# jjalcaraz-upct/network-slicing

Hardware: AMD Instinct MI355X
Metric: env-steps/sec (batched RanSlice.step, scenario_0) (higher is better)
Workload: dtype f64

## Files before the change

network-slicing_amd/csrc/rs_api.hip:

```cpp

#include <hip/hip_runtime.h>

#include <cmath>
#include <cstdio>
#include <cstdlib>
#include <cstring>
#include <string>
#include <vector>

#include "rs_host.h"

#ifdef RS_DEV
static inline const char* dev_env(const char* name) { return getenv(name); }
#else
static inline const char* dev_env(const char*) { return nullptr; }
#endif

#include "rs_embb.hip"
#include "rs_mmtc.hip"
#include "rs_order.hip"
#include "rs_mux.hip"

using namespace rs;

// ... 285 lines not shown
    for (int k = 0; k < 4; ++k) atomicAdd(&acc[k], loc[k]);
    __syncthreads();
    if (threadIdx.x < 4) atomicAdd((unsigned long long*)&out[threadIdx.x], acc[threadIdx.x]);
}

}


static void mcs_factors(double* A, double* B) {
    double Delta = 0.1;
    double a = 1.0 / Delta;
    double s01 = rs_sigmoid(0.1, 0.0, 1.0), s09 = rs_sigmoid(0.9, 0.0, 1.0);
    a = a * (rs_log(1.0 / s01 - 1.0) - rs_log(1.0 / s09 - 1.0));
    *A = a;
    *B = -rs_log(1.0 / s09 - 1.0);
}

static void mcs_lookup(const rs_config* c, double A, double B, int e_snr, int* mcs_out, int* rate_out) {
    double rx_prob = 1.0 - 0.1;
    int mcs;
    for (mcs = 0; mcs < c->n_mcs; ++mcs) {
        double x = A * ((double)e_snr - c->mcs_snr[mcs]) - B;
        if (rs_sigmoid(x, 0.0, 1.0) < rx_prob) {
            *mcs_out = mcs - 1 > 0 ? mcs - 1 : 0;
            *rate_out = (int)((double)c->sym_per_prb * (c->mcs_rate[mcs] * (double)c->mcs_order[mcs]));
            return;
        }
    }
    mcs = c->n_mcs - 1;
    *mcs_out = mcs;
    *rate_out = (int)((double)c->sym_per_prb * (c->mcs_rate[mcs] * (double)c->mcs_order[mcs]));
}

static void rx_fast_setup(RsDev& d, double* band0) {
    const double A = d.mcsA;
    double kmax = 0.0, kmin = 1e300;
    bool ok = std::isfinite(A) && A > 0.0 && std::isfinite(d.mcsB);
    for (int m = 0; m < 3; ++m) {
        const double k = d.mi_k[m];
        ok = ok && std::isfinite(k) && k > 0.0 && std::isfinite(d.mi_x0[m]);
        kmax = k > kmax ? k : kmax;
        kmin = k < kmin ? k : kmin;
        d.rx_c1[m] = (float)(-k * RS_INV_LN2);
    }
    ok = ok && A / kmax >= 1.0 && A / kmin <= 1.0e4;
    d.rx_invA = ok ? (float)(1.0 / A) : 0.0f;
    d.rx_B = (float)d.mcsB;
    d.rx_band = 0.0;
    *band0 = ok ? 6.0e-6 + 6.0e-6 * (kmax / A) : 0.0;
    d.rx_band1 = ok ? 4.0e-5 / A + 1.0e-6 : 0.0;
    if (dev_env("RANSLICE_RX_EXACT")) *band0 = 0.0;
    if (const char* e = dev_env("RANSLICE_RX_BAND_SCALE")) {
        const double f = atof(e);
        if (f >= 1.0) d.rx_band1 *= f;
    }
}

extern "C" int rs_create(const rs_config* cfg, int device, rs_handle** out) {
    if (!cfg || !out) return RS_EINVAL;
    *out = nullptr;
    rs_handle* h = new rs_handle();
    *out = h;
    h->cfg = *cfg;
    h->device = device;
    if (cfg->n_envs <= 0 || cfg->n_prbs <= 0 || cfg->n_prbs > RS_MAX_PRBS || cfg->n_embb < 0 || cfg->n_mmtc < 0 ||
        cfg->n_embb + cfg->n_mmtc <= 0 || cfg->slots_per_step <= 0 || cfg->slots_per_step > 63 || cfg->n_mcs <= 0 || cfg->n_mcs > 32 ||
// ... 280 lines not shown
        vbytes += h->valid_host[f].size();
        bool any_valid = false;
        for (uint8_t v : h->valid_host[f]) {
            if (!v) d.has_nan = 1;
            any_valid = any_valid || v;
        }
        if (!any_valid) {
            h->err = "rs_load_fading: a trace has no NaN-free column";
            return RS_EINVAL;
        }
    }
    if (elems + (size_t)RS_MAX_PRBS >= (size_t)1 << 31) {
        h->err = "rs_load_fading: tables exceed 2^31 samples";
        return RS_EINVAL;
    }
    if (h->fad) (void)hipFree(h->fad);
    if (h->fad_valid) (void)hipFree(h->fad_valid);
    if (h->fad32) (void)hipFree(h->fad32);
    if (h->fps) (void)hipFree(h->fps);
    h->fad32 = nullptr;
    h->fps = nullptr;
    HIPCHK(h, hipMalloc((void**)&h->fad, sizeof(double) * (elems + 16)));
    HIPCHK(h, hipMalloc((void**)&h->fad_valid, vbytes + 16));
    if (const char* v = dev_env("RANSLICE_GUARD"))
        if (v[0] == '2') fprintf(stderr, "RANSLICE_GUARD: fading table at %p, %zu bytes\n", (void*)h->fad, sizeof(double) * (elems + 16));
    for (int f = 0; f < RS_N_TRACES; ++f) {
        HIPCHK(h, hipMemcpyAsync(h->fad + d.fad_off[f], h->fad_host[f].data(), sizeof(double) * h->fad_host[f].size(),
                                 hipMemcpyHostToDevice, h->stream));
        HIPCHK(h, hipMemcpyAsync(h->fad_valid + d.valid_off[f], h->valid_host[f].data(), h->valid_host[f].size(),
                                 hipMemcpyHostToDevice, h->stream));
    }
    {
        const int P = d.P;
        std::vector<float> t32(elems + 64, 0.0f);
        std::vector<double> ps((elems / (size_t)P) * (size_t)(P + 1) + 16, 0.0);
        double smax = 0.0;
        bool finite = true;
        for (int f = 0; f < RS_N_TRACES; ++f) {
            const std::vector<double>& tab = h->fad_host[f];
            const size_t cols = tab.size() / (size_t)P, c0 = (size_t)d.fad_off[f] / (size_t)P;
            d.col_off[f] = (int32_t)c0;
            for (size_t t = 0; t < cols; ++t) {
                long double acc = 0.0L;
                double* row = &ps[(c0 + t) * (size_t)(P + 1)];
                row[0] = 0.0;
                const bool ok = h->valid_host[f][t] != 0;
                for (int p = 0; p < P; ++p) {
                    const double v = tab[t * (size_t)P + p];
                    t32[(size_t)d.fad_off[f] + t * (size_t)P + p] = (float)v;
                    acc += (long double)v;
                    row[p + 1] = (double)acc;
                    if (ok) {
                        finite = finite && std::isfinite(v);
                        smax = std::fabs(v) > smax ? std::fabs(v) : smax;
                    }
                }
            }
        }
        const bool small = finite && smax <= 1.0e3;
        const bool ps_fits = ps.size() + (size_t)RS_MAX_PRBS < ((size_t)1 << 31);
        d.est_band = (small && ps_fits && !dev_env("RANSLICE_EST_EXACT")) ? 1.0e-9 : 0.0;
        double kmax = 0.0;
        for (int m = 0; m < 3; ++m) kmax = d.mi_k[m] > kmax ? d.mi_k[m] : kmax;
        d.rx_band = (small && h->rx_band0 > 0.0) ? h->rx_band0 + 0.5 * kmax * 5.97e-8 * smax : 0.0;
        if (const char* e = dev_env("RANSLICE_RX_BAND_SCALE")) {
            const double fsc = atof(e);
            if (fsc >= 1.0) d.rx_band *= fsc;
        }
        if (const char* e = dev_env("RANSLICE_EST_BAND")) {
            const double b = atof(e);
            if (d.est_band > 0.0 && b > 0.0 && b < 0.5) d.est_band = b;
        }
        HIPCHK(h, hipMalloc((void**)&h->fad32, sizeof(float) * t32.size()));
        HIPCHK(h, hipMalloc((void**)&h->fps, sizeof(double) * ps.size()));
        HIPCHK(h, hipMemcpy(h->fad32, t32.data(), sizeof(float) * t32.size(), hipMemcpyHostToDevice));
        HIPCHK(h, hipMemcpy(h->fps, ps.data(), sizeof(double) * ps.size(), hipMemcpyHostToDevice));
    }
    HIPCHK(h, hipMemcpyAsync(h->ddev, &d, sizeof d, hipMemcpyHostToDevice, h->stream));
    HIPCHK(h, hipStreamSynchronize(h->stream));
    h->fad_hash = fading_hash(h);
    for (int f = 0; f < RS_N_TRACES; ++f) {
        std::vector<double>().swap(h->fad_host[f]);
        std::vector<uint8_t>().swap(h->valid_host[f]);
    }
    return RS_OK;
}

extern "C" int rs_load_fading(rs_handle* h, int trace_id, const double* data, int rows, int cols) {
    if (!h) return RS_EINVAL;
    if (trace_id < 0 || trace_id >= RS_N_TRACES || !data || rows <= 0 || cols <= 0 || h->cfg.n_prbs > 2 * rows) {
        h->err = "rs_load_fading: bad arguments";
        return RS_EINVAL;
    }
    HIPCHK(h, hipSetDevice(h->device));
    drop_graph(h);
    if (h->tables_borrowed) {
        h->err = "rs_load_fading: a lookahead branch handle shares its tables";
        return RS_ESTATE;
    }
    if (h->la) {
        HIPCHK(h, hipStreamSynchronize(h->stream));
        rs_destroy(h->la);
        h->la = nullptr;
    }
    h->fad_hash = 0;
    const int P = h->cfg.n_prbs > rows ? h->cfg.n_prbs : rows;
    if (h->hdev.P != 0 && h->hdev.P != P) {
        h->err = "rs_load_fading: all traces must have the same number of rows";
// ... 610 lines not shown
```

network-slicing_amd/csrc/rs_device.h:

```cpp
#pragma once
#include <stdint.h>

#define RS_GROUP 32
#define RS_BURSTS 16
#define RS_BURST_MAX_LEN 16000
#define RS_LUT_MAX 64
#define RS_NEVER 0x7fffffff
#define RS_MAX_PRBS 256

#define rs_burst_code(end_abs) (0x8000u | ((unsigned)(end_abs) & 0x7fffu))
#define rs_burst_rel(code, now) ((int)(((((unsigned)(code)) - (unsigned)(now)) & 0x7fffu) ^ 0x4000u) - 0x4000)

struct RsDev {
    int32_t n_envs, n_prbs, n_embb, n_mmtc, n_slices, slots, n_vars;
    int32_t n_act;
    int32_t mux;
    int32_t P;
    int32_t T[3];
    int32_t has_nan;
    int64_t fad_off[3];
    int64_t valid_off[3];
    double slot_length;
    double cbr_bits;
    double cbr_ia_scale, cbr_hold_scale;
    double vbr_ia_scale, vbr_hold_scale;
    double vbr_p_size, vbr_b_size, vbr_inter;
    double sla[6], norm[10];
    double prop_A, prop_B;
    double mcsA, mcsB;
    double pf_a, pf_b;
    double slot_rc;
    int32_t pf_div_fast;
    int32_t gran;
    int32_t lut_lo, lut_n;
    int32_t lut_mcs[RS_LUT_MAX], lut_rate[RS_LUT_MAX];
    double mcs_ref[32];
    int32_t mcs_mod[32];
    double mi_x0[3], mi_k[3];
    double rx_band;
    double est_band;
    int32_t col_off[3];
    int32_t pad_rx;
    double rx_band1;
    float rx_c1[3];
    float rx_invA, rx_B;
    double penalty;
    int32_t mtc_n_dev, mtc_cap, mtc_n_rep, mtc_n_period;
    int32_t mtc_rep_set[8], mtc_period_set[8];
    double sla_mtc_delay, norm_mmtc[3];
};

struct RsState {
    int32_t* t_n_ue;
    int32_t* t_cbr_at;
    int32_t* t_vbr_at;
    uint32_t* t_ctr;
    uint32_t* t_serial;
    int32_t* t_cost;
    double* u_queue;
    double* u_th;
    double* u_nominal;
    int32_t* u_hold_at;
    int32_t* u_e_snr;
    int32_t* u_findex;
    int32_t* u_bits;
    int32_t* u_prbs;
    int32_t* u_vbr_at;
    uint32_t* u_ctr;
    uint32_t* u_serial;
    int32_t* u_flags;
    uint16_t* u_burst;
    uint64_t* seeds;
    int32_t* err;
};
```

network-slicing_amd/csrc/rs_embb.hip:

```cpp

#pragma once
#include <hip/hip_runtime.h>
#include <stdint.h>

#include "rs_device.h"

#if defined(__HIP_DEVICE_COMPILE__)
__device__ double rs_exp_ool(double x);
__device__ double rs_log_ool(double x);
#define RS_EXP_CALL rs_exp_ool
#define RS_LOG_CALL rs_log_ool
#endif
#include "../../include/rs_philox.h"
#include "../../include/ranslice.h"

typedef double rs_d2 __attribute__((ext_vector_type(2)));
#if defined(__HIP_DEVICE_COMPILE__)
__device__ __noinline__ double rs_exp_ool(double x) { return rs_exp(x); }
__device__ __noinline__ double rs_log_ool(double x) { return rs_log(x); }
__device__ __forceinline__ double rs_exp_sel(double x, double core) {
    double v = x < -745.2 ? 0.0 : core;
    v = x > 709.782712893384 ? rs_inf() : v;
    return x != x ? x : v;
}
// ... 73 lines not shown
#define SEC_FLUSH(buf)                                                                                  \
    if ((threadIdx.x & 63u) == 0u) {                                                                    \
        unsigned long long tot_ = 0;                                                                    \
        for (int i_ = 0; i_ < 13; ++i_) tot_ += sec_acc[i_];                                            \
        for (int i_ = 0; i_ < 16; ++i_)                                                                 \
            if (i_ != 14) atomicAdd((unsigned long long*)&(buf)[i_], sec_acc[i_]);                      \
         \
        if (tot_ > atomicMax((unsigned long long*)&(buf)[14], tot_))                                    \
            for (int i_ = 0; i_ < 16; ++i_) (buf)[16 + 4 * (size_t)n_tasks + i_] = sec_acc[i_];        \
    }                                                                                                   \
    if ((threadIdx.x & 63u) != 0u && sec_acc[13]) atomicAdd((unsigned long long*)&(buf)[13], sec_acc[13]); \
    if (gl == 0 && valid) {  \
        unsigned long long tot_ = 0;                                                                    \
        for (int i_ = 0; i_ < 13; ++i_) tot_ += sec_acc[i_];                                            \
        (buf)[16 + task * 4 + 0] = tot_;                                                                \
         \
        (buf)[16 + task * 4 + 1] = (unsigned long long)S.t_n_ue[task] |                                 \
                                   ((unsigned long long)__builtin_amdgcn_s_getreg(63508) << 32);        \
        (buf)[16 + task * 4 + 2] = (unsigned long long)A.actions[rep * n_slices + sl] |                 \
                                   ((unsigned long long)__builtin_amdgcn_s_getreg(63492) << 32);        \
        (buf)[16 + task * 4 + 3] = (unsigned long long)(stat >> 18) | ((sec_t0 - tot_) << 24);  \
    }
#else
#define SEC_DECL
#define SEC_MARK(i)
#define SEC_FLUSH(buf)
#endif

__device__ __forceinline__ int bperm(int v, int src_lane) {
    return __builtin_amdgcn_ds_bpermute(src_lane << 2, v);
}
__device__ __forceinline__ unsigned bperm(unsigned v, int src_lane) {
    return (unsigned)__builtin_amdgcn_ds_bpermute(src_lane << 2, (int)v);
}
__device__ __forceinline__ double bperm(double v, int src_lane) {
    uint64_t u = rs_d2u(v);
    int lo = __builtin_amdgcn_ds_bpermute(src_lane << 2, (int)(uint32_t)u);
    int hi = __builtin_amdgcn_ds_bpermute(src_lane << 2, (int)(uint32_t)(u >> 32));
    return rs_u2d(((uint64_t)(uint32_t)hi << 32) | (uint32_t)lo);
}

__device__ __forceinline__ bool wave_any(bool c) { return __builtin_amdgcn_ballot_w64(c) != 0ull; }

#define DPP_XOR1 0xB1
#define DPP_XOR2 0x4E
#define DPP_HMIRROR 0x141
#define DPP_MIRROR 0x140
#define DPP_BCAST15 0x142

template <int CTRL>
__device__ __forceinline__ int dpp_i(int v) {
    return __builtin_amdgcn_mov_dpp(v, CTRL, 0xF, 0xF, false);
}
template <int CTRL>
__device__ __forceinline__ double dpp_d(double v) {
    uint64_t u = rs_d2u(v);
    int lo = __builtin_amdgcn_mov_dpp((int)(uint32_t)u, CTRL, 0xF, 0xF, false);
    int hi = __builtin_amdgcn_mov_dpp((int)(uint32_t)(u >> 32), CTRL, 0xF, 0xF, false);
    return rs_u2d(((uint64_t)(uint32_t)hi << 32) | (uint32_t)lo);
}
__device__ __forceinline__ double max_finite(double a, double b) {
    double r;
    asm("v_max_f64 %0, %1, %2\n\ts_nop 1" : "=v"(r) : "v"(a), "v"(b));
    return r;
}

// ... 352 lines not shown
        const int n = __builtin_amdgcn_readlane(rbs, ol);
        const int c0 = __builtin_amdgcn_readlane(span_col, ol);
        const int md = __builtin_amdgcn_readlane(mod, ol);
        const double nom = nom_wave[ol];
        const double x0 = mi[md], kk = mi[4 + md];
        for (int k0 = 0; k0 < n; k0 += 128) {
            const int k1 = k0 + lane, k2 = k0 + 64 + lane;
            const double x1 = (k1 < n ? fad[c0 + k1] : 0.0) + nom, x2 = (k2 < n ? fad[c0 + k2] : 0.0) + nom;
            const rs_d2 sg = rs_sigmoid2(x1, x2, x0, kk);
            if (k1 < n) wmi[k1] = sg.x;
            if (k2 < n) wmi[k2] = sg.y;
        }
        __builtin_amdgcn_wave_barrier();
        const double sv = team_pairwise(n, lane & 7, lane < 8, [&](int i1, bool p1, int i2, bool p2) {
            rs_d2 o;
            o.x = p1 ? wmi[i1] : 0.0;
            o.y = p2 ? wmi[i2] : 0.0;
            return o;
        });
        const double got = bperm(sv, 0);
        if (lane == ol) out = got;
        __builtin_amdgcn_wave_barrier();
    }
    return out;
}

__device__ __forceinline__ float fast_sigmoid(float v, float hi, float c1, float loc) {
    const float t2 = __builtin_fmaf(v + hi, c1, loc);
    const float e = __builtin_amdgcn_exp2f(t2);
    return __builtin_amdgcn_rcpf(1.0f + e);
}
#define RS_RX_LF(u) (0.6931471805599453f * __builtin_amdgcn_logf((float)(1.0 - (u)) * __builtin_amdgcn_rcpf((float)(u))))
#define RS_RX_DQ(D, lf) (((D)->rx_B - (lf)) * (D)->rx_invA)
typedef float rs_f4u __attribute__((ext_vector_type(4), aligned(4)));
__device__ __forceinline__ float fast_quad(rs_f4u q, int k0, int n, float hi, float c1, float loc) {
    const float s0 = fast_sigmoid(q.x, hi, c1, loc), s1 = fast_sigmoid(q.y, hi, c1, loc);
    const float s2 = fast_sigmoid(q.z, hi, c1, loc), s3 = fast_sigmoid(q.w, hi, c1, loc);
    return ((k0 < n ? s0 : 0.0f) + (k0 + 1 < n ? s1 : 0.0f)) + ((k0 + 2 < n ? s2 : 0.0f) + (k0 + 3 < n ? s3 : 0.0f));
}

#define RS_FAST_WIDE 64
template <bool TEAMC, class F>
__device__ __forceinline__ double fast_team_sums(const double* mi, const float* c1s, const float* fad32, const double* nom_wave,
                                                 bool mine, int rbs, int span_col, int mod, F meanwhile) {
    const int lane = (int)(threadIdx.x & 63u);
    double out = 0.0;
    const unsigned long long wmask = __builtin_amdgcn_ballot_w64(mine);
    const int n_sp = __popcll(wmask);
    const int my_sp = __popcll(wmask & ((1ull << lane) - 1ull));
    const int team = lane >> 3, j = lane & 7;
    unsigned long long rest = wmask;
    for (int round = 0; round * 8 < n_sp; ++round) {
        int owner = 0;
#pragma unroll
        for (int k = 0; k < 8; ++k) {
            const int o = rest ? __builtin_ctzll(rest) : 0;
            rest &= rest - 1ull;
            owner = (TEAMC ? team_is(k) : team == k) ? o : owner;
        }
        const bool on = round * 8 + team < n_sp;
        const int c0 = bperm(span_col, owner);
        const int n_o = bperm(rbs, owner);
        const int n = on ? n_o : 0;
        const int md = bperm(mod, owner);
        const float* __restrict__ sp = fad32 + (on ? c0 : 0) + 4 * j;
        rs_f4u qa = {0.0f, 0.0f, 0.0f, 0.0f}, qb = {0.0f, 0.0f, 0.0f, 0.0f};
        if (4 * j < n) qa = *(const rs_f4u*)sp;
        if (32 + 4 * j < n) qb = *(const rs_f4u*)(sp + 32);
        const double nomx = nom_wave[owner] - mi[md];
        const float c1 = c1s[md];
        if (round == 0) meanwhile();
        const float hi = (float)nomx, loc = (float)(nomx - (double)hi) * c1;
        double acc = (double)fast_quad(qa, 4 * j, n, hi, c1, loc);
        if (wave_any(n > 32)) acc += (double)fast_quad(qb, 32 + 4 * j, n, hi, c1, loc);
        acc += dpp_d<DPP_XOR1>(acc);
        acc += dpp_d<DPP_XOR2>(acc);
        acc += dpp_d<DPP_HMIRROR>(acc);
        const double got = bperm(acc, (my_sp & 7) << 3);
        if (mine && (my_sp >> 3) == round) out = got;
    }
    return out;
}

__device__ __forceinline__ double fast_wide_sums(const double* mi, const float* c1s, const float* fad32, const double* nom_wave,
                                                 bool mine, int rbs, int span_col, int mod) {
    const int lane = (int)(threadIdx.x & 63u);
    double out = 0.0;
    unsigned long long wm = __builtin_amdgcn_ballot_w64(mine);
    rs_f4u q = {0.0f, 0.0f, 0.0f, 0.0f};
    {
        const int ol = __builtin_ctzll(wm);
        if (4 * lane < __builtin_amdgcn_readlane(rbs, ol)) q = *(const rs_f4u*)(fad32 + __builtin_amdgcn_readlane(span_col, ol) + 4 * lane);
    }
    while (wm != 0ull) {
        const int ol = __builtin_ctzll(wm);
        wm &= wm - 1ull;
        const int n = __builtin_amdgcn_readlane(rbs, ol);
        const int md = __builtin_amdgcn_readlane(mod, ol);
        rs_f4u qn = {0.0f, 0.0f, 0.0f, 0.0f};
        if (wm != 0ull) {
            const int on_ = __builtin_ctzll(wm);
            if (4 * lane < __builtin_amdgcn_readlane(rbs, on_)) qn = *(const rs_f4u*)(fad32 + __builtin_amdgcn_readlane(span_col, on_) + 4 * lane);
        }
        const double nomx = nom_wave[ol] - mi[md];
        const float c1 = c1s[md];
        const float hi = (float)nomx, loc = (float)(nomx - (double)hi) * c1;
        double acc = (double)fast_quad(q, 4 * lane, n, hi, c1, loc);
        acc += dpp_d<DPP_XOR1>(acc);
        acc += dpp_d<DPP_XOR2>(acc);
        acc += dpp_d<DPP_HMIRROR>(acc);
        acc += dpp_d<DPP_MIRROR>(acc);
        acc += bperm(acc, lane ^ 16);
        acc += bperm(acc, lane ^ 32);
        if (lane == ol) out = acc;
        q = qn;
    }
    return out;
}

template <int G, bool TRACE, bool BLOCK, bool FDIV>
__global__ __launch_bounds__(256, (G == 16 && !TRACE) ? RS_OCC : RS_OCC_OTHER) void embb_step_kernel(StepArgs A) {
    static_assert(G == 8 || G == 16 || G == 32, "lanes per task");
    constexpr bool TABLE = !BLOCK;
    constexpr bool TEAMC = !BLOCK;
    constexpr int TPB = 256 / G;
    constexpr int TPW = 64 / G;
    constexpr int CH = 12;
    __shared__ unsigned short L_burst[RS_BURSTS][256];
    __shared__ int L_hold[256];
    __shared__ int L_uvbr[256];
    __shared__ unsigned L_serial[256], L_ctr[256];
    __shared__ int L_acc_traf[256], L_acc_bits[256], L_acc_prbs[256];
    __shared__ double L_nom[256];
    __shared__ short T_esnr[256][CH];
    __shared__ int L_lut[RS_LUT_MAX];
    __shared__ double L_ref[32];
    __shared__ double L_mi[8];
    __shared__ float L_c1[4];
    __shared__ TraceRow L_tr[4];
    __shared__ int L_task[TPB][4];
    __shared__ double W_mi[4][RS_WIDE_MAX];
    const RsDev* __restrict__ D = A.D;
    const int tid = (int)threadIdx.x;
    if (tid < RS_LUT_MAX) L_lut[tid] = tid < D->lut_n ? ((D->mcs_mod[D->lut_mcs[tid]] << 24) | (D->lut_mcs[tid] << 16) | D->lut_rate[tid]) : 0;
    if (tid >= 64 && tid < 96) L_ref[tid - 64] = D->mcs_ref[tid - 64];
    if (tid >= 96 && tid < 104) L_mi[tid - 96] = (tid & 3) == 3 ? 0.0 : (tid < 100 ? D->mi_x0[tid - 96] : D->mi_k[tid - 100]);
    if (tid >= 104 && tid < 108) L_c1[tid - 104] = tid < 107 ? D->rx_c1[tid - 104] : 0.0f;
    if (TABLE && tid >= 112 && tid < 116) {
        const int f = tid - 112;
        TraceRow tr = {0, 0, 0, 0};
        if (f < RS_N_TRACES) tr = {D->T[f], D->col_off[f], (int)D->fad_off[f], (int)D->valid_off[f]};
        L_tr[f] = tr;
    }
    __syncthreads();
    const RsState& S = *A.S;
    const int clock0 = (int)A.run[0];
    const int lane = (int)(threadIdx.x & 63u);
    const int gl = lane & (G - 1);
    const int gbase = lane & ~(G - 1);
    const int tb = tid - gl;
    const int wb = tid & ~63;
    const int tq = tid / G;
    const int n_tasks = D->n_envs * D->n_embb;
    int task = A.spread ? (int)blockIdx.x * 4 + (int)(threadIdx.x >> 6) : (int)blockIdx.x * TPB + (int)(threadIdx.x / G);
    const int n_mine = A.order_cnt >= 0 ? A.order_cnt : n_tasks;
    const bool in_range = task < n_mine && (!A.spread || gbase == 0);
    if (!in_range) task = n_mine - 1;
    if (A.order) task = A.order[A.order_off + task];
    const bool selected = in_range && (!A.replay || A.redo[task] != 0);
    if (!wave_any(selected)) return;
    const int rep = task / D->n_embb;
    const int sl = task - rep * D->n_embb;
    const int n_slices = D->n_slices;
    const int P = D->P;
    const double slot_len = D->slot_length;
    const double pf_a = D->pf_a, pf_b = D->pf_b;
    const double slot_rc = D->slot_rc;
    constexpr bool pf_div_fast = FDIV;
#define RS_TRACE_ROW(ft) (TABLE ? L_tr[ft] : TraceRow{0, 0, 0, 0})
#define RS_TR(ft, row, field, a, b, c) (TABLE ? (row).field : sel3(ft, a, b, c))
// ... 683 lines not shown
            }

            SEC_MARK(3)
            const int prb_i = group_excl_scan<G>(rbs, gl);
            const bool needed = sched && active && rbs > 0 && (TRACE || bits > 0);
            const int span_col = col + prb_lo + prb_i;
            bool exact = needed;
            bool rx_ok = false;
            if (!TRACE) n_rx_tests += (unsigned)__popcll(__builtin_amdgcn_ballot_w64(needed));
            if (!TRACE && rx_fast) {
                const bool single = rbs == 1;
                const bool multi = needed && !single;
                const bool fw = multi && rbs > RS_FAST_WIDE;
                const double x0 = L_mi[mod], ref = L_ref[mcs];
                double S1 = 0.0;
                if (needed && single) S1 = A.fad[span_col];
                bool central = false;
                double St = 0.0;
                auto threshold = [&]() {
                    double u = 0.5;
                    if (needed) {
                        rs_stream st = {key0, key1, (uint32_t)sl, L_serial[lt], L_ctr[lt]};
                        u = rs_stream_uniform(&st);
                    }
                    central = u >= 1.0e-4 && u <= 1.0 - 1.0e-4;
                    const float lf = RS_RX_LF(u);
                    const float dq = RS_RX_DQ(D, lf);
                    const float ystar = fast_sigmoid((float)((ref - x0) + (double)dq), 0.0f, L_c1[mod], 0.0f);
                    St = single ? (double)dq : (double)rbs * (double)ystar;
                };
                double S = 0.0;
                bool thr_done = false;
                if (wave_any(multi && !fw)) {
                    S = fast_team_sums<TEAMC>(L_mi, L_c1, A.fad32, &L_nom[wb], multi && !fw, rbs, span_col, mod, threshold);
                    thr_done = true;
                }
                if (wave_any(fw)) {
                    const double s2 = fast_wide_sums(L_mi, L_c1, A.fad32, &L_nom[wb], fw, rbs, span_col, mod);
                    S = fw ? s2 : S;
                }
                if (!thr_done) threshold();
                if (needed && single) S = (S1 + L_nom[lt]) - ref;
                const double band = single ? D->rx_band1 : (double)rbs * D->rx_band;
                const double dd = S - St;
                const bool sure = central && (dd > band || dd < -band);
                rx_ok = dd > 0.0;
                exact = needed && !sure;
            }
            SEC_MARK(10)
            if (wave_any(exact)) {
                double sum_rx = 0.0;
                constexpr int WIDE = RS_WIDE_SPAN;
                const bool wide_sp = exact && rbs > WIDE && rbs <= RS_WIDE_MAX;
                if (wave_any(wide_sp)) sum_rx = wide_response(L_mi, A.fad, W_mi[tid >> 6], &L_nom[wb], wide_sp, rbs, span_col, mod);
                sum_rx = team_response<TEAMC>(L_mi, A.fad, &L_nom[wb], exact && !wide_sp, rbs, span_col, mod, sum_rx);
                if (exact) {
                    const double x0 = L_mi[mod], kk = L_mi[4 + mod];
                    double s_eff = sum_rx;
                    if (rbs > 1) s_eff = rs_inv_sigmoid(sum_rx / (double)rbs, x0, kk);
                    const double x = D->mcsA * (s_eff - L_ref[mcs]) - D->mcsB;
                    p_rx = rs_sigmoid(x, 0.0, 1.0);
                    if (!TRACE) atomicAdd((unsigned long long*)&A.counters[(size_t)task * 4 + 1], 1ull);
                }
            }
            SEC_MARK(4)
            if (sched && active) {
                bool received = false;
                if (rbs > 0) {
                    const unsigned c = L_ctr[lt];
                    if (exact) {
                        rs_stream st = {key0, key1, (uint32_t)sl, L_serial[lt], c};
// ... 163 lines not shown
```

network-slicing_amd/csrc/rs_probe.hip:

```cpp

enum {
    RSP_EXP_OOL = 0, RSP_EXP_INLINE, RSP_EXP_NONPOS, RSP_EXP2_OOL, RSP_LOG_OOL, RSP_LOG_INLINE, RSP_LOG10, RSP_ACOS,
    RSP_SIGMOID, RSP_SIGMOID2, RSP_INV_SIGMOID, RSP_DIV, RSP_SQRT, RSP_RINT, RSP_FMA,
    RSP_PHILOX, RSP_UNIFORM, RSP_EXPONENTIAL, RSP_INTEGERS, RSP_PM1, RSP_NORMAL, RSP_WALKER, RSP_MACRO_CELL,
    RSP_LANE_PAIRWISE, RSP_TEAM_PAIRWISE, RSP_FAST_SIGMOID, RSP_RX_DQ, RSP_N_OPS
};

struct ProbeArgs {
    const void* in;
    void* out;
    int64_t n;
    const RsDev* D;
    double p[4];
    float f[4];
};

template <int OP>
__global__ __launch_bounds__(256) void probe_kernel(ProbeArgs a) {
#if defined(__HIP_DEVICE_COMPILE__)
    const int64_t i = (int64_t)blockIdx.x * 256 + (int64_t)threadIdx.x;
    const bool live = i < a.n;
    const int64_t e = live ? i : 0;
    const double* in = (const double*)a.in;
    double* out = (double*)a.out;
    if constexpr (OP <= RSP_RINT && OP != RSP_EXP2_OOL && OP != RSP_SIGMOID2 && OP != RSP_DIV) {
        const double x = in[e];
        double y;
        if constexpr (OP == RSP_EXP_OOL) y = rs_exp_ool(x);
        if constexpr (OP == RSP_EXP_INLINE) y = rs_exp(x);
        if constexpr (OP == RSP_EXP_NONPOS) y = rs_exp_nonpos(x);
        if constexpr (OP == RSP_LOG_OOL) y = rs_log_ool(x);
        if constexpr (OP == RSP_LOG_INLINE) y = rs_log(x);
        if constexpr (OP == RSP_LOG10) y = rs_log10(x);
        if constexpr (OP == RSP_ACOS) y = rs_acos(x);
        if constexpr (OP == RSP_SIGMOID) y = rs_sigmoid(x, a.p[0], a.p[1]);
        if constexpr (OP == RSP_INV_SIGMOID) y = rs_inv_sigmoid(x, a.p[0], a.p[1]);
        if constexpr (OP == RSP_SQRT) y = RS_SQRT(x);
        if constexpr (OP == RSP_RINT) y = RS_RINT(x);
// ... 48 lines not shown
            ((int32_t*)a.out)[2 * i] = findex;
            ((int32_t*)a.out)[2 * i + 1] = fstep;
        }
    } else if constexpr (OP == RSP_MACRO_CELL) {
        const uint32_t* w = (const uint32_t*)a.in + 5 * e;
        const rs_stream st = {w[0], w[1], w[2], w[3], w[4]};
        const MacroCell mc = macro_cell_draw(a.D, st);
        if (live) {
            out[2 * i] = mc.x;
            out[2 * i + 1] = mc.y;
        }
    } else if constexpr (OP == RSP_LANE_PAIRWISE) {
        const int32_t* w = (const int32_t*)a.in + 2 * e;
        const double* vec = (const double*)((const int32_t*)a.in + 2 * a.n);
        const int len = live ? w[0] : 0;
        const double* __restrict__ colp = vec + (live ? w[1] : 0);
        const double s = lane_pairwise(len, len > 0, [&](int k) { return colp[k]; });
        if (live) out[i] = s;
    } else if constexpr (OP == RSP_TEAM_PAIRWISE) {
        const int64_t team = e >> 3;
        const int j = (int)(threadIdx.x & 7u);
        const int32_t* w = (const int32_t*)a.in + 2 * team;
        const double* vec = (const double*)((const int32_t*)a.in + 2 * (a.n >> 3));
        const int len = live ? w[0] : 0;
        const bool on = len > 0;
        const double* __restrict__ sp = vec + (on ? w[1] : 0);
        const double s = team_pairwise(len, j, on, [&](int i1, bool p1, int i2, bool p2) {
            rs_d2 o;
            o.x = p1 ? sp[i1] : 0.0;
            o.y = p2 ? sp[i2] : 0.0;
            return o;
        });
        if (live && j == 0) out[team] = s;
    } else if constexpr (OP == RSP_FAST_SIGMOID) {
        const double nomx = a.p[2] - a.p[0];
        const float c1 = a.f[0];
        const float hi = (float)nomx, loc = (float)(nomx - (double)hi) * c1;
        const float y = fast_sigmoid(((const float*)a.in)[e], hi, c1, loc);
        if (live) ((float*)a.out)[i] = y;
    } else if constexpr (OP == RSP_RX_DQ) {
        const double u = in[e];
        const RsDev* D = a.D;
        const float lf = RS_RX_LF(u);
        const float dq = RS_RX_DQ(D, lf);
        if (live) ((float*)a.out)[i] = dq;
    }
#endif
}

extern "C" int rs_dev_probe(int device, int op, const void* in, void* out, int64_t n, const double* params) {
    if (op < 0 || op >= RSP_N_OPS || n <= 0 || n > ((int64_t)1 << 22) || !in || !out) return RS_EINVAL;
    ProbeArgs a;
    memset(&a, 0, sizeof a);
    a.n = n;
    for (int k = 0; k < 4; ++k) a.p[k] = params ? params[k] : 0.0;
    size_t in_bytes = 8 * (size_t)n, out_bytes = 8 * (size_t)n, in_pad = 0;
    bool needs_params = false;
    switch (op) {
        case RSP_SIGMOID: case RSP_INV_SIGMOID: needs_params = true; break;
        case RSP_EXP2_OOL: out_bytes = 16 * (size_t)n; break;
        case RSP_SIGMOID2: out_bytes = 16 * (size_t)n; needs_params = true; break;
        case RSP_DIV: in_bytes = 16 * (size_t)n; break;
        case RSP_FMA: in_bytes = 24 * (size_t)n; break;
        case RSP_PHILOX: in_bytes = 24 * (size_t)n; break;
        case RSP_WALKER: in_bytes = 24 * (size_t)n; needs_params = true; break;
        case RSP_UNIFORM: case RSP_PM1: in_bytes = 20 * (size_t)n; out_bytes = 16 * (size_t)n; break;
        case RSP_EXPONENTIAL: case RSP_INTEGERS: case RSP_NORMAL: case RSP_MACRO_CELL:
            in_bytes = 20 * (size_t)n;
            out_bytes = 16 * (size_t)n;
            needs_params = true;
            break;
        case RSP_LANE_PAIRWISE: case RSP_TEAM_PAIRWISE: needs_params = true; break;
        case RSP_FAST_SIGMOID: in_bytes = out_bytes = 4 * (size_t)n; needs_params = true; break;
        case RSP_RX_DQ: out_bytes = 4 * (size_t)n; needs_params = true; break;
        default: break;
    }
    if (needs_params && !params) return RS_EINVAL;
    if (op == RSP_INTEGERS && !(a.p[0] >= 1.0 && a.p[0] <= 9.0e15)) return RS_EINVAL;
    if (op == RSP_WALKER && !(a.p[0] >= 1.0 && a.p[0] <= 2147483647.0)) return RS_EINVAL;
    if (op == RSP_LANE_PAIRWISE || op == RSP_TEAM_PAIRWISE) {
        if (!(a.p[0] >= 1.0 && a.p[0] <= (double)(1 << 24))) return RS_EINVAL;
        const int64_t m = (int64_t)a.p[0];
        if (op == RSP_TEAM_PAIRWISE && (n & 7)) return RS_EINVAL;
        const int64_t rows = op == RSP_TEAM_PAIRWISE ? n >> 3 : n;
        const int32_t* w = (const int32_t*)in;
        for (int64_t r = 0; r < rows; ++r)
            if (w[2 * r] < 0 || w[2 * r] > 256 || w[2 * r + 1] < 0 || (int64_t)w[2 * r + 1] + w[2 * r] > m) return RS_EINVAL;
        in_pad = 64 * 8;
        in_bytes = 8 * (size_t)rows + 8 * (size_t)m;
        out_bytes = 8 * (size_t)rows;
    }
    RsDev* hd = new RsDev();
    memset(hd, 0, sizeof *hd);
    if (op == RSP_FAST_SIGMOID || op == RSP_RX_DQ) {
        const bool fs = op == RSP_FAST_SIGMOID;
        hd->mcsA = fs ? a.p[1] : a.p[0];
        hd->mcsB = fs ? 0.0 : a.p[1];
        for (int m = 0; m < 3; ++m) {
            hd->mi_k[m] = fs ? a.p[1] : a.p[0];
            hd->mi_x0[m] = fs ? a.p[0] : 0.0;
        }
        double band0 = 0.0;
        rx_fast_setup(*hd, &band0);
        a.f[0] = hd->rx_c1[0];
        if (hd->rx_invA == 0.0f) {
            delete hd;
            return RS_EINVAL;
        }
    } else if (op == RSP_MACRO_CELL) {
        hd->prop_A = a.p[0];
        hd->prop_B = a.p[1];
    }
    int ndev = 0;
    if (hipGetDeviceCount(&ndev) != hipSuccess || device < 0 || device >= ndev || hipSetDevice(device) != hipSuccess) {
        delete hd;
        return RS_EHIP;
    }
    void *d_in = nullptr, *d_out = nullptr;
    RsDev* d_dev = nullptr;
    int rc = RS_EHIP;
    do {
        if (hipMalloc(&d_in, in_bytes + in_pad) != hipSuccess || hipMalloc(&d_out, out_bytes) != hipSuccess) break;
        if (in_pad && hipMemset((char*)d_in + in_bytes, 0, in_pad) != hipSuccess) break;
        if (hipMemcpy(d_in, in, in_bytes, hipMemcpyHostToDevice) != hipSuccess) break;
        if (hipMemset(d_out, 0, out_bytes) != hipSuccess) break;
        if (op == RSP_MACRO_CELL || op == RSP_RX_DQ) {
            if (hipMalloc((void**)&d_dev, sizeof(RsDev)) != hipSuccess ||
                hipMemcpy(d_dev, hd, sizeof(RsDev), hipMemcpyHostToDevice) != hipSuccess)
                break;
            a.D = d_dev;
        }
        a.in = d_in;
        a.out = d_out;
        const dim3 grid((unsigned)((n + 255) / 256)), block(256);
        switch (op) {
#define RSP_CASE(OP) case OP: hipLaunchKernelGGL(probe_kernel<OP>, grid, block, 0, 0, a); break;
            RSP_CASE(RSP_EXP_OOL) RSP_CASE(RSP_EXP_INLINE) RSP_CASE(RSP_EXP_NONPOS) RSP_CASE(RSP_EXP2_OOL) RSP_CASE(RSP_LOG_OOL)
            RSP_CASE(RSP_LOG_INLINE) RSP_CASE(RSP_LOG10) RSP_CASE(RSP_ACOS) RSP_CASE(RSP_SIGMOID) RSP_CASE(RSP_SIGMOID2)
            RSP_CASE(RSP_INV_SIGMOID) RSP_CASE(RSP_DIV) RSP_CASE(RSP_SQRT) RSP_CASE(RSP_RINT) RSP_CASE(RSP_FMA) RSP_CASE(RSP_PHILOX)
            RSP_CASE(RSP_UNIFORM) RSP_CASE(RSP_EXPONENTIAL) RSP_CASE(RSP_INTEGERS) RSP_CASE(RSP_PM1) RSP_CASE(RSP_NORMAL)
            RSP_CASE(RSP_WALKER) RSP_CASE(RSP_MACRO_CELL) RSP_CASE(RSP_LANE_PAIRWISE) RSP_CASE(RSP_TEAM_PAIRWISE)
            RSP_CASE(RSP_FAST_SIGMOID) RSP_CASE(RSP_RX_DQ)
#undef RSP_CASE
            default: break;
        }
        if (hipGetLastError() != hipSuccess) break;
        if (hipDeviceSynchronize() != hipSuccess) break;
        if (hipMemcpy(out, d_out, out_bytes, hipMemcpyDeviceToHost) != hipSuccess) break;
        rc = RS_OK;
    } while (0);
    delete hd;
    if (d_in) (void)hipFree(d_in);
    if (d_out) (void)hipFree(d_out);
    if (d_dev) (void)hipFree(d_dev);
    if (hipDeviceSynchronize() != hipSuccess) rc = RS_EHIP;
    return rc;
}
```

Baseline: 4.907 million.

## Precompute per-modulation exp2 tables of fading to turn sigmoid into fma+rcp

Fading values are now stored alongside three precomputed tables exp2(-k/ln2 * v), one per modulation, built once at fading-table upload. In the eMBB inner sigmoid sum, each element is then computed as rcp(1 + c*E), where c is a per-slice coefficient derived once per slice. This replaces a per-element float exp/sigmoid evaluation with an fma and a reciprocal. The wide-sum path is moved out of line, presumably to reduce register pressure. In exchange the fading table takes four times the device memory and bandwidth, and large exponents can lose precision or overflow in float.

```diff
diff --git a/network-slicing_amd/csrc/rs_api.hip b/network-slicing_amd/csrc/rs_api.hip
--- a/network-slicing_amd/csrc/rs_api.hip
+++ b/network-slicing_amd/csrc/rs_api.hip
@@ -341,6 +341,9 @@
     *rate_out = (int)((double)c->sym_per_prb * (c->mcs_rate[mcs] * (double)c->mcs_order[mcs]));
 }
 
+static inline double rx_slope(double k) { return -k * RS_INV_LN2; }
+static inline float rx_exp_entry(double v, double s1) { return (float)std::exp2(s1 * v); }
+
 static void rx_fast_setup(RsDev& d, double* band0) {
     const double A = d.mcsA;
     double kmax = 0.0, kmin = 1e300;
@@ -687,7 +690,10 @@
     }
     {
         const int P = d.P;
-        std::vector<float> t32(elems + 64, 0.0f);
+        const size_t stride = elems + 64;
+        std::vector<float> t32(4 * stride, 0.0f);
+        const double s1[3] = {rx_slope(d.mi_k[0]), rx_slope(d.mi_k[1]), rx_slope(d.mi_k[2])};
+        d.fexp_stride = (int32_t)stride;
         std::vector<double> ps((elems / (size_t)P) * (size_t)(P + 1) + 16, 0.0);
         double smax = 0.0;
         bool finite = true;
@@ -702,7 +708,9 @@
                 const bool ok = h->valid_host[f][t] != 0;
                 for (int p = 0; p < P; ++p) {
                     const double v = tab[t * (size_t)P + p];
-                    t32[(size_t)d.fad_off[f] + t * (size_t)P + p] = (float)v;
+                    const size_t e = (size_t)d.fad_off[f] + t * (size_t)P + p;
+                    t32[e] = (float)v;
+                    for (int m = 0; m < 3; ++m) t32[(m + 1) * stride + e] = rx_exp_entry(v, s1[m]);
                     acc += (long double)v;
                     row[p + 1] = (double)acc;
                     if (ok) {
@@ -727,8 +735,8 @@
             if (d.est_band > 0.0 && b > 0.0 && b < 0.5) d.est_band = b;
         }
         HIPCHK(h, hipMalloc((void**)&h->fad32, sizeof(float) * t32.size()));
+        HIPCHK(h, hipMemcpy(h->fad32, t32.data(), sizeof(float) * t32.size(), hipMemcpyHostToDevice));
         HIPCHK(h, hipMalloc((void**)&h->fps, sizeof(double) * ps.size()));
-        HIPCHK(h, hipMemcpy(h->fad32, t32.data(), sizeof(float) * t32.size(), hipMemcpyHostToDevice));
         HIPCHK(h, hipMemcpy(h->fps, ps.data(), sizeof(double) * ps.size(), hipMemcpyHostToDevice));
     }
     HIPCHK(h, hipMemcpyAsync(h->ddev, &d, sizeof d, hipMemcpyHostToDevice, h->stream));
diff --git a/network-slicing_amd/csrc/rs_device.h b/network-slicing_amd/csrc/rs_device.h
--- a/network-slicing_amd/csrc/rs_device.h
+++ b/network-slicing_amd/csrc/rs_device.h
@@ -40,7 +40,7 @@
     double rx_band;
     double est_band;
     int32_t col_off[3];
-    int32_t pad_rx;
+    int32_t fexp_stride;
     double rx_band1;
     float rx_c1[3];
     float rx_invA, rx_B;
diff --git a/network-slicing_amd/csrc/rs_embb.hip b/network-slicing_amd/csrc/rs_embb.hip
--- a/network-slicing_amd/csrc/rs_embb.hip
+++ b/network-slicing_amd/csrc/rs_embb.hip
@@ -129,6 +129,9 @@
 }
 __device__ __forceinline__ unsigned bperm(unsigned v, int src_lane) {
     return (unsigned)__builtin_amdgcn_ds_bpermute(src_lane << 2, (int)v);
+}
+__device__ __forceinline__ float bperm(float v, int src_lane) {
+    return __builtin_bit_cast(float, __builtin_amdgcn_ds_bpermute(src_lane << 2, __builtin_bit_cast(int, v)));
 }
 __device__ __forceinline__ double bperm(double v, int src_lane) {
     uint64_t u = rs_d2u(v);
@@ -547,16 +550,112 @@
 }
 #define RS_RX_LF(u) (0.6931471805599453f * __builtin_amdgcn_logf((float)(1.0 - (u)) * __builtin_amdgcn_rcpf((float)(u))))
 #define RS_RX_DQ(D, lf) (((D)->rx_B - (lf)) * (D)->rx_invA)
+__device__ __forceinline__ float fast_sigmoid_tab(float E, float c) {
+    return __builtin_amdgcn_rcpf(__builtin_fmaf(c, E, 1.0f));
+}
+__device__ __forceinline__ float fast_coef(double nomx, double s1) {
+    const double t = nomx * s1;
+    const int n = (int)t;
+    const float c = __builtin_ldexpf(__builtin_amdgcn_exp2f((float)(t - (double)n)), n);
+    return __builtin_fabs(t) <= 64.0 ? c : __builtin_nanf("");
+}
 typedef float rs_f4u __attribute__((ext_vector_type(4), aligned(4)));
-__device__ __forceinline__ float fast_quad(rs_f4u q, int k0, int n, float hi, float c1, float loc) {
+__device__ __forceinline__ float fast_quad(rs_f4u q, int k0, int n, float c) {
+    const float s0 = fast_sigmoid_tab(q.x, c), s1 = fast_sigmoid_tab(q.y, c);
+    const float s2 = fast_sigmoid_tab(q.z, c), s3 = fast_sigmoid_tab(q.w, c);
+    return ((k0 < n ? s0 : 0.0f) + (k0 + 1 < n ? s1 : 0.0f)) + ((k0 + 2 < n ? s2 : 0.0f) + (k0 + 3 < n ? s3 : 0.0f));
+}
+
+#define RS_FAST_WIDE 64
+template <bool TEAMC, class F>
+__device__ __forceinline__ double fast_team_sums(const double* mi, const float* fexp, int estride, const double* nom_wave,
+                                                 bool mine, int rbs, int span_col, int mod, F meanwhile) {
+    const int lane = (int)(threadIdx.x & 63u);
+    double out = 0.0;
+    const unsigned long long wmask = __builtin_amdgcn_ballot_w64(mine);
+    const int n_sp = __popcll(wmask);
+    const int my_sp = __popcll(wmask & ((1ull << lane) - 1ull));
+    const int team = lane >> 3, j = lane & 7;
+    unsigned long long rest = wmask;
+    const float c_own = fast_coef(nom_wave[lane] - mi[mod], mi[8 + mod]);
+    for (int round = 0; round * 8 < n_sp; ++round) {
+        int owner = 0;
+#pragma unroll
+        for (int k = 0; k < 8; ++k) {
+            const int o = rest ? __builtin_ctzll(rest) : 0;
+            rest &= rest - 1ull;
+            owner = (TEAMC ? team_is(k) : team == k) ? o : owner;
+        }
+        const bool on = round * 8 + team < n_sp;
+        const int c0 = bperm(span_col, owner);
+        const int n_o = bperm(rbs, owner);
+        const int n = on ? n_o : 0;
+        const int md = bperm(mod, owner);
+        const float c = bperm(c_own, owner);
+        const float* __restrict__ sp = fexp + (size_t)(unsigned)(md + 1) * (size_t)(unsigned)estride + (on ? c0 : 0) + 4 * j;
+        rs_f4u qa = {0.0f, 0.0f, 0.0f, 0.0f}, qb = {0.0f, 0.0f, 0.0f, 0.0f};
+        if (4 * j < n) qa = *(const rs_f4u*)sp;
+        if (32 + 4 * j < n) qb = *(const rs_f4u*)(sp + 32);
+        if (round == 0) meanwhile();
+        double acc = (double)fast_quad(qa, 4 * j, n, c);
+        if (wave_any(n > 32)) acc += (double)fast_quad(qb, 32 + 4 * j, n, c);
+        acc += dpp_d<DPP_XOR1>(acc);
+        acc += dpp_d<DPP_XOR2>(acc);
+        acc += dpp_d<DPP_HMIRROR>(acc);
+        const double got = bperm(acc, (my_sp & 7) << 3);
+        if (mine && (my_sp >> 3) == round) out = got;
+    }
+    return out;
+}
+
+__device__ __forceinline__ double fast_wide_sums(const double* mi, const float* fexp, int estride, const double* nom_wave,
+                                                 bool mine, int rbs, int span_col, int mod) {
+    const int lane = (int)(threadIdx.x & 63u);
+    double out = 0.0;
+    unsigned long long wm = __builtin_amdgcn_ballot_w64(mine);
+    rs_f4u q = {0.0f, 0.0f, 0.0f, 0.0f};
+    {
+        const int ol = __builtin_ctzll(wm);
+        const float* tab = fexp + (size_t)(unsigned)(__builtin_amdgcn_readlane(mod, ol) + 1) * (size_t)(unsigned)estride;
+        if (4 * lane < __builtin_amdgcn_readlane(rbs, ol)) q = *(const rs_f4u*)(tab + __builtin_amdgcn_readlane(span_col, ol) + 4 * lane);
+    }
+    while (wm != 0ull) {
+        const int ol = __builtin_ctzll(wm);
+        wm &= wm - 1ull;
+        const int n = __builtin_amdgcn_readlane(rbs, ol);
+        rs_f4u qn = {0.0f, 0.0f, 0.0f, 0.0f};
+        if (wm != 0ull) {
+            const int on_ = __builtin_ctzll(wm);
+            const float* tab = fexp + (size_t)(unsigned)(__builtin_amdgcn_readlane(mod, on_) + 1) * (size_t)(unsigned)estride;
+            if (4 * lane < __builtin_amdgcn_readlane(rbs, on_)) qn = *(const rs_f4u*)(tab + __builtin_amdgcn_readlane(span_col, on_) + 4 * lane);
+        }
+        const int md = __builtin_amdgcn_readlane(mod, ol);
+        const float c = fast_coef(nom_wave[ol] - mi[md], mi[8 + md]);
+        double acc = (double)fast_quad(q, 4 * lane, n, c);
+        acc += dpp_d<DPP_XOR1>(acc);
+        acc += dpp_d<DPP_XOR2>(acc);
+        acc += dpp_d<DPP_HMIRROR>(acc);
+        acc += dpp_d<DPP_MIRROR>(acc);
+        acc += bperm(acc, lane ^ 16);
+        acc += bperm(acc, lane ^ 32);
+        if (lane == ol) out = acc;
+        q = qn;
+    }
+    return out;
+}
+__device__ __noinline__ double fast_wide_sums_ool(const double* mi, const float* fexp, int estride, const double* nom_wave,
+                                                  bool mine, int rbs, int span_col, int mod) {
+    return fast_wide_sums(mi, fexp, estride, nom_wave, mine, rbs, span_col, mod);
+}
+
+__device__ __forceinline__ float fast_quad_f32(rs_f4u q, int k0, int n, float hi, float c1, float loc) {
     const float s0 = fast_sigmoid(q.x, hi, c1, loc), s1 = fast_sigmoid(q.y, hi, c1, loc);
     const float s2 = fast_sigmoid(q.z, hi, c1, loc), s3 = fast_sigmoid(q.w, hi, c1, loc);
     return ((k0 < n ? s0 : 0.0f) + (k0 + 1 < n ? s1 : 0.0f)) + ((k0 + 2 < n ? s2 : 0.0f) + (k0 + 3 < n ? s3 : 0.0f));
 }
 
-#define RS_FAST_WIDE 64
 template <bool TEAMC, class F>
-__device__ __forceinline__ double fast_team_sums(const double* mi, const float* c1s, const float* fad32, const double* nom_wave,
+__device__ __forceinline__ double fast_team_sums_f32(const double* mi, const float* c1s, const float* fad32, const double* nom_wave,
                                                  bool mine, int rbs, int span_col, int mod, F meanwhile) {
     const int lane = (int)(threadIdx.x & 63u);
     double out = 0.0;
@@ -586,8 +685,8 @@
         const float c1 = c1s[md];
         if (round == 0) meanwhile();
         const float hi = (float)nomx, loc = (float)(nomx - (double)hi) * c1;
-        double acc = (double)fast_quad(qa, 4 * j, n, hi, c1, loc);
-        if (wave_any(n > 32)) acc += (double)fast_quad(qb, 32 + 4 * j, n, hi, c1, loc);
+        double acc = (double)fast_quad_f32(qa, 4 * j, n, hi, c1, loc);
+        if (wave_any(n > 32)) acc += (double)fast_quad_f32(qb, 32 + 4 * j, n, hi, c1, loc);
         acc += dpp_d<DPP_XOR1>(acc);
         acc += dpp_d<DPP_XOR2>(acc);
         acc += dpp_d<DPP_HMIRROR>(acc);
@@ -597,7 +696,7 @@
     return out;
 }
 
-__device__ __forceinline__ double fast_wide_sums(const double* mi, const float* c1s, const float* fad32, const double* nom_wave,
+__device__ __forceinline__ double fast_wide_sums_f32(const double* mi, const float* c1s, const float* fad32, const double* nom_wave,
                                                  bool mine, int rbs, int span_col, int mod) {
     const int lane = (int)(threadIdx.x & 63u);
     double out = 0.0;
@@ -620,7 +719,7 @@
         const double nomx = nom_wave[ol] - mi[md];
         const float c1 = c1s[md];
         const float hi = (float)nomx, loc = (float)(nomx - (double)hi) * c1;
-        double acc = (double)fast_quad(q, 4 * lane, n, hi, c1, loc);
+        double acc = (double)fast_quad_f32(q, 4 * lane, n, hi, c1, loc);
         acc += dpp_d<DPP_XOR1>(acc);
         acc += dpp_d<DPP_XOR2>(acc);
         acc += dpp_d<DPP_HMIRROR>(acc);
@@ -638,6 +737,7 @@
     static_assert(G == 8 || G == 16 || G == 32, "lanes per task");
     constexpr bool TABLE = !BLOCK;
     constexpr bool TEAMC = !BLOCK;
+    constexpr bool EXPTAB = !BLOCK;
     constexpr int TPB = 256 / G;
     constexpr int TPW = 64 / G;
     constexpr int CH = 12;
@@ -650,7 +750,7 @@
     __shared__ short T_esnr[256][CH];
     __shared__ int L_lut[RS_LUT_MAX];
     __shared__ double L_ref[32];
-    __shared__ double L_mi[8];
+    __shared__ double L_mi[12];
     __shared__ float L_c1[4];
     __shared__ TraceRow L_tr[4];
     __shared__ int L_task[TPB][4];
@@ -661,6 +761,7 @@
     if (tid >= 64 && tid < 96) L_ref[tid - 64] = D->mcs_ref[tid - 64];
     if (tid >= 96 && tid < 104) L_mi[tid - 96] = (tid & 3) == 3 ? 0.0 : (tid < 100 ? D->mi_x0[tid - 96] : D->mi_k[tid - 100]);
     if (tid >= 104 && tid < 108) L_c1[tid - 104] = tid < 107 ? D->rx_c1[tid - 104] : 0.0f;
+    if (tid >= 108 && tid < 112) L_mi[8 + tid - 108] = tid < 111 ? -D->mi_k[tid - 108] * RS_INV_LN2 : 0.0;
     if (TABLE && tid >= 112 && tid < 116) {
         const int f = tid - 112;
         TraceRow tr = {0, 0, 0, 0};
@@ -1410,11 +1511,18 @@
                 double S = 0.0;
                 bool thr_done = false;
                 if (wave_any(multi && !fw)) {
-                    S = fast_team_sums<TEAMC>(L_mi, L_c1, A.fad32, &L_nom[wb], multi && !fw, rbs, span_col, mod, threshold);
+                    if constexpr (EXPTAB)
+                        S = fast_team_sums<TEAMC>(L_mi, A.fad32, D->fexp_stride, &L_nom[wb], multi && !fw, rbs, span_col, mod, threshold);
+                    else
+                        S = fast_team_sums_f32<TEAMC>(L_mi, L_c1, A.fad32, &L_nom[wb], multi && !fw, rbs, span_col, mod, threshold);
                     thr_done = true;
                 }
                 if (wave_any(fw)) {
-                    const double s2 = fast_wide_sums(L_mi, L_c1, A.fad32, &L_nom[wb], fw, rbs, span_col, mod);
+                    double s2;
+                    if constexpr (EXPTAB)
+                        s2 = fast_wide_sums_ool(L_mi, A.fad32, D->fexp_stride, &L_nom[wb], fw, rbs, span_col, mod);
+                    else
+                        s2 = fast_wide_sums_f32(L_mi, L_c1, A.fad32, &L_nom[wb], fw, rbs, span_col, mod);
                     S = fw ? s2 : S;
                 }
                 if (!thr_done) threshold();
diff --git a/network-slicing_amd/csrc/rs_probe.hip b/network-slicing_amd/csrc/rs_probe.hip
--- a/network-slicing_amd/csrc/rs_probe.hip
+++ b/network-slicing_amd/csrc/rs_probe.hip
@@ -3,7 +3,7 @@
     RSP_EXP_OOL = 0, RSP_EXP_INLINE, RSP_EXP_NONPOS, RSP_EXP2_OOL, RSP_LOG_OOL, RSP_LOG_INLINE, RSP_LOG10, RSP_ACOS,
     RSP_SIGMOID, RSP_SIGMOID2, RSP_INV_SIGMOID, RSP_DIV, RSP_SQRT, RSP_RINT, RSP_FMA,
     RSP_PHILOX, RSP_UNIFORM, RSP_EXPONENTIAL, RSP_INTEGERS, RSP_PM1, RSP_NORMAL, RSP_WALKER, RSP_MACRO_CELL,
-    RSP_LANE_PAIRWISE, RSP_TEAM_PAIRWISE, RSP_FAST_SIGMOID, RSP_RX_DQ, RSP_N_OPS
+    RSP_LANE_PAIRWISE, RSP_TEAM_PAIRWISE, RSP_FAST_SIGMOID, RSP_RX_DQ, RSP_FAST_SIGMOID64, RSP_N_OPS
 };
 
 struct ProbeArgs {
@@ -118,11 +118,9 @@
             return o;
         });
         if (live && j == 0) out[team] = s;
-    } else if constexpr (OP == RSP_FAST_SIGMOID) {
-        const double nomx = a.p[2] - a.p[0];
-        const float c1 = a.f[0];
-        const float hi = (float)nomx, loc = (float)(nomx - (double)hi) * c1;
-        const float y = fast_sigmoid(((const float*)a.in)[e], hi, c1, loc);
+    } else if constexpr (OP == RSP_FAST_SIGMOID || OP == RSP_FAST_SIGMOID64) {
+        const float c = fast_coef(a.p[2] - a.p[0], a.p[3]);
+        const float y = fast_sigmoid_tab(((const float*)a.in)[e], c);
         if (live) ((float*)a.out)[i] = y;
     } else if constexpr (OP == RSP_RX_DQ) {
         const double u = in[e];
@@ -157,7 +155,7 @@
             needs_params = true;
             break;
         case RSP_LANE_PAIRWISE: case RSP_TEAM_PAIRWISE: needs_params = true; break;
-        case RSP_FAST_SIGMOID: in_bytes = out_bytes = 4 * (size_t)n; needs_params = true; break;
+        case RSP_FAST_SIGMOID: case RSP_FAST_SIGMOID64: in_bytes = out_bytes = 4 * (size_t)n; needs_params = true; break;
         case RSP_RX_DQ: out_bytes = 4 * (size_t)n; needs_params = true; break;
         default: break;
     }
@@ -178,8 +176,9 @@
     }
     RsDev* hd = new RsDev();
     memset(hd, 0, sizeof *hd);
-    if (op == RSP_FAST_SIGMOID || op == RSP_RX_DQ) {
-        const bool fs = op == RSP_FAST_SIGMOID;
+    std::vector<float> entries;
+    if (op == RSP_FAST_SIGMOID || op == RSP_FAST_SIGMOID64 || op == RSP_RX_DQ) {
+        const bool fs = op != RSP_RX_DQ;
         hd->mcsA = fs ? a.p[1] : a.p[0];
         hd->mcsB = fs ? 0.0 : a.p[1];
         for (int m = 0; m < 3; ++m) {
@@ -188,10 +187,16 @@
         }
         double band0 = 0.0;
         rx_fast_setup(*hd, &band0);
-        a.f[0] = hd->rx_c1[0];
         if (hd->rx_invA == 0.0f) {
             delete hd;
             return RS_EINVAL;
+        }
+        if (fs) {
+            a.p[3] = rx_slope(a.p[1]);
+            entries.resize((size_t)n);
+            for (int64_t i = 0; i < n; ++i)
+                entries[(size_t)i] = rx_exp_entry(op == RSP_FAST_SIGMOID ? (double)((const float*)in)[i] : ((const double*)in)[i], a.p[3]);
+            in = entries.data();
         }
     } else if (op == RSP_MACRO_CELL) {
         hd->prop_A = a.p[0];
@@ -226,7 +231,7 @@
             RSP_CASE(RSP_INV_SIGMOID) RSP_CASE(RSP_DIV) RSP_CASE(RSP_SQRT) RSP_CASE(RSP_RINT) RSP_CASE(RSP_FMA) RSP_CASE(RSP_PHILOX)
             RSP_CASE(RSP_UNIFORM) RSP_CASE(RSP_EXPONENTIAL) RSP_CASE(RSP_INTEGERS) RSP_CASE(RSP_PM1) RSP_CASE(RSP_NORMAL)
             RSP_CASE(RSP_WALKER) RSP_CASE(RSP_MACRO_CELL) RSP_CASE(RSP_LANE_PAIRWISE) RSP_CASE(RSP_TEAM_PAIRWISE)
-            RSP_CASE(RSP_FAST_SIGMOID) RSP_CASE(RSP_RX_DQ)
+            RSP_CASE(RSP_FAST_SIGMOID) RSP_CASE(RSP_RX_DQ) RSP_CASE(RSP_FAST_SIGMOID64)
 #undef RSP_CASE
             default: break;
         }
```

Result: no change. 4.920 million, median of 6 (+0.3%).
